# Membrizard/ml_conformer_generator

Hardware: AMD Instinct MI355X
Metric: valid molecules/sec @100 diffusion steps (`value` = RAW molecules/s through the whole public path: the reference's validity gate needs RDKit + trained weights, unavailable offline; see `validity`) (higher is better)
Workload: dtype f32

## Files before the change

### ml_conformer_generator_amd/csrc/mcg_gemm_kernels.h

```cpp
#pragma once
#include "mcg_gemm.h"

#include <type_traits>


__device__ __forceinline__ float* mcg_gemm_c_ptr(const McgGemmArgs& p, int orow, int nt, int g) {
    if (!p.c_blocked) return p.C + (size_t)orow * p.ldc + nt * 16 + 4 * g;
    const int part = nt >= 27 ? 1 : 0, ntp = nt - 27 * part;
    return p.C + ((size_t)((part * 14 + (ntp >> 1)) * 8 + (ntp & 1) * 4 + g) * p.M + orow) * 4;
}

__device__ __forceinline__ void mcg_gemm_side_job(const McgGemmArgs& p, int block) {
    const int idx = block * 256 + (int)threadIdx.x;
    const int v = idx >> 2, comp = idx & 3;
    if (v < p.side_M && comp < 3) {
        const int4 sl = p.side_slots[v];
        p.side_x[(size_t)v * 4 + comp] += (((p.side_u[(size_t)sl.x * 4 + comp] + p.side_u[(size_t)sl.y * 4 + comp]) + p.side_u[(size_t)sl.z * 4 + comp]) +
                                           p.side_u[(size_t)sl.w * 4 + comp]) / 100.0f;
    }
}

template <int RN, int GATHER = 0>
__global__ __launch_bounds__(256) void mcg_gemm_bf16_kernel(McgGemmArgs p) {
    const int lane = threadIdx.x & 63;
// ... 213 lines not shown
            if (k0 + e >= K) v[e] = 0.f;
        typedef __bf16 bf16x4 __attribute__((ext_vector_type(4)));
        const bf16x4 h4 = (bf16x4){(__bf16)v[0], (__bf16)v[1], (__bf16)v[2], (__bf16)v[3]};
        char* dst = reinterpret_cast<char*>(sA) + (((2 * frag_kb + (i >> 1)) * 64 + 16 * (piece >> 1) + 8 * (i & 1) + prow) * 16 + (piece & 1) * 8);
        *reinterpret_cast<bf16x4*>(dst) = h4;
    };
    {
        const __amdgpu_buffer_rsrc_t rs_a1 = __builtin_amdgcn_make_buffer_rsrc(const_cast<float*>(p.A1), 0, 0xffffffff, 0x00020000);
        for (int kb = wid; kb < b1; kb += MCG_LDSG_WAVES) {
            f32x4 v[4];
#pragma unroll
            for (int i = 0; i < 4; ++i) v[i] = __builtin_bit_cast(f32x4, ld(rs_a1, (unsigned)(qrow[i] * p.lda1 + 32 * kb + 4 * piece) * 4u, 0));
#pragma unroll
            for (int i = 0; i < 4; ++i) park_quarter(kb, i, v[i], 32 * kb + 4 * piece, p.K1);
        }
    }
    constexpr int NS = GATHER >= 2 ? GATHER : 1;
    constexpr int S2P = SEG2 ? MCG_LDSG_S2P : 0;
    f32x4 s2[SEG2 ? 2 : 1][4][NS];
    const __amdgpu_buffer_rsrc_t rs_a2 = __builtin_amdgcn_make_buffer_rsrc(const_cast<float*>(p.A2 ? p.A2 : p.A1), 0, 0xffffffff, 0x00020000);
    int srow[4][NS];
#pragma unroll
    for (int i = 0; i < 4; ++i) {
        if constexpr (GATHER >= 2) {
            const int4 sl = (SEG2 && p.a2_rows) ? p.a2_rows[qrow[i]] : (int4){0, 0, 0, 0};
            const int rows[4] = {sl.x, sl.y, sl.z, sl.w};
#pragma unroll
            for (int q = 0; q < NS; ++q) srow[i][q] = rows[q];
        } else {
            srow[i][0] = qrow[i];
        }
    }
    auto seg2_issue = [&](int j) {
        int kb = wid + j * MCG_LDSG_WAVES;
        kb = kb < b2 ? kb : b2 - 1;
#pragma unroll
        for (int i = 0; i < 4; ++i)
#pragma unroll
            for (int q = 0; q < NS; ++q)
                s2[j][i][q] = __builtin_bit_cast(f32x4, ld(rs_a2, (unsigned)(srow[i][q] * p.lda2 + 32 * kb + 4 * piece) * 4u, 0));
    };
    auto seg2_park = [&](int j) {
        const int kb = wid + j * MCG_LDSG_WAVES;
        if (kb >= b2) return;
#pragma unroll
        for (int i = 0; i < 4; ++i) {
            f32x4 v = s2[j][i][0];
            if constexpr (GATHER >= 2) {
#pragma unroll
                for (int q = 1; q < NS; ++q) v += s2[j][i][q];
#pragma unroll
                for (int e = 0; e < 4; ++e) v[e] = mcg_div100(v[e]);
            }
            park_quarter(b1 + kb, i, v, 32 * kb + 4 * piece, p.K2);
        }
    };
    f32x4 eres[RESID ? 2 : 1][RN];
    if constexpr (RESID) {
#pragma unroll
        for (int n = 0; n < RN; ++n) {
            const int col = ncl[n] * 16 + 4 * g;
#pragma unroll
            for (int m = 0; m < 2; ++m) {
                const int orow = row0 + 16 * m + c;
                eres[m][n] = (orow < p.M && col + 3 < p.n_store) ? *reinterpret_cast<const f32x4*>(p.resid + (size_t)orow * p.ldr + col)
                                                                  : (f32x4){0.f, 0.f, 0.f, 0.f};
            }
        }
    }
    constexpr bool OVERLAP2 = SEG2 && GATHER <= 2;
    if (SEG2 && b2 > 0) {
        if constexpr (OVERLAP2) {
#pragma unroll
            for (int j = 0; j < S2P; ++j) seg2_issue(j);
        } else {
#pragma unroll
            for (int j = 0; j < S2P; ++j) { seg2_issue(j); seg2_park(j); }
        }
    }
    asm volatile("s_waitcnt lgkmcnt(0)\n\ts_barrier" ::: "memory");

    f32x4 acc[2][RN];
#pragma unroll
    for (int m = 0; m < 2; ++m)
#pragma unroll
        for (int n = 0; n < RN; ++n) acc[m][n] = (f32x4){0.f, 0.f, 0.f, 0.f};
    auto compute = [&](int slot, int kb) {
        const bf16x8 A0 = sA[(2 * kb) * 64 + lane];
        const bf16x8 A1 = sA[(2 * kb + 1) * 64 + lane];
#pragma unroll
        for (int n = 0; n < RN; ++n) {
            acc[0][n] = mcg_mfma_bf16(Br[slot][n], A0, acc[0][n]);
            acc[1][n] = mcg_mfma_bf16(Br[slot][n], A1, acc[1][n]);
        }
    };
    auto k_loop = [&](int k0, int k1) {
        int kb = k0;
#pragma unroll 1
        for (; kb + RING <= k1; kb += RING) {
#pragma unroll
            for (int r = 0; r < RING; ++r) {
                compute(r, kb + r); __builtin_amdgcn_sched_barrier(0); load_w(r, kb + r + RING); __builtin_amdgcn_sched_barrier(0);
            }
        }
#pragma unroll
        for (int r = 0; r < RING - 1; ++r)
            if (kb + r < k1) compute(r, kb + r);
    };
    if (SEG2 && b2 > 0 && OVERLAP2) {
        k_loop(0, b1);
#pragma unroll
        for (int r = 0; r < RING; ++r) load_w(r, b1 + r);
#pragma unroll
        for (int j = 0; j < S2P; ++j) seg2_park(j);
        asm volatile("s_waitcnt lgkmcnt(0)\n\ts_barrier" ::: "memory");
        k_loop(b1, blocks);
    } else {
        k_loop(0, blocks);
    }

#pragma unroll
    for (int n = 0; n < RN; ++n) {
        if (!nvalid[n]) continue;
        const int col = (nt0 + n) * 16 + 4 * g;
        if (col >= p.n_store) continue;
        const f32x4 ebias = p.bias ? *reinterpret_cast<const f32x4*>(p.bias + col) : (f32x4){0.f, 0.f, 0.f, 0.f};
#pragma unroll
        for (int m = 0; m < 2; ++m) {
            const int orow = row0 + 16 * m + c;
            if (orow >= p.M) continue;
            f32x4 v = acc[m][n] + ebias;
            if (p.act == MCG_ACT_SILU) {
#pragma unroll
                for (int r = 0; r < 4; ++r) v[r] = mcg_silu(v[r]);
            } else if (p.act == MCG_ACT_RELU) {
#pragma unroll
                for (int r = 0; r < 4; ++r) v[r] = fmaxf(v[r], 0.f);
            }
            if constexpr (RESID) v += eres[m][n];
            float* dst = mcg_gemm_c_ptr(p, orow, nt0 + n, g);
            if (col + 3 < p.n_store) {
                *reinterpret_cast<f32x4*>(dst) = v;
            } else {
#pragma unroll
                for (int r = 0; r < 4; ++r)
                    if (col + r < p.n_store) dst[r] = v[r];
            }
        }
    }
}

typedef __bf16 bf16x4 __attribute__((ext_vector_type(4)));

template <int RN>
__global__ __launch_bounds__(256) void mcg_gemm_x6_kernel(McgGemmArgs p) {
    __shared__ __attribute__((aligned(16))) uint16_t a_lds[2 * 2 * 3 * 64 * 8];
    const int lane = threadIdx.x & 63;
    const int wid = __builtin_amdgcn_readfirstlane(threadIdx.x >> 6);
    const int g = lane >> 4, c = lane & 15;
    const int wave_cols = (p.n_tiles + RN - 1) / RN;
    const int col_groups = (wave_cols + 3) / 4;
    const int blk = mcg_xcd_remap(blockIdx.x, gridDim.x);
    const int row0 = (blk / col_groups) * 32;
    const int wcol = (blk % col_groups) * 4 + wid;
    const bool wave_live = wcol < wave_cols;
    const int nt0 = (wave_live ? wcol : wave_cols - 1) * RN;
    bool nvalid[RN];
    int ncl[RN];
#pragma unroll
    for (int n = 0; n < RN; ++n) {
        nvalid[n] = wave_live && nt0 + n < p.n_tiles;
        ncl[n] = nt0 + n < p.n_tiles ? n : 0;
    }
    f32x4 acc[2][RN];
#pragma unroll
    for (int m = 0; m < 2; ++m)
#pragma unroll
        for (int n = 0; n < RN; ++n) acc[m][n] = (f32x4){0.f, 0.f, 0.f, 0.f};
    f32x4 ebias[RN];
    f32x4 eres[2][RN];
#pragma unroll
    for (int n = 0; n < RN; ++n) {
        const int col = (nt0 + ncl[n]) * 16 + 4 * g;
        ebias[n] = p.bias ? *reinterpret_cast<const f32x4*>(p.bias + col) : (f32x4){0.f, 0.f, 0.f, 0.f};
#pragma unroll
        for (int m = 0; m < 2; ++m) {
            const int orow = row0 + 16 * m + c;
            eres[m][n] = (p.resid && orow < p.M && col + 3 < p.n_store) ? *reinterpret_cast<const f32x4*>(p.resid + (size_t)orow * p.ldr + col)
                                                                        : (f32x4){0.f, 0.f, 0.f, 0.f};
        }
    }
    const int my_row = 8 * wid + (lane >> 3), my_k = 4 * (lane & 7);
    const int src_row = row0 + my_row < p.M ? row0 + my_row : p.M - 1;
    const int frag_off = (((my_row >> 4) * 3) * 64 + ((my_k >> 3) * 16 + (my_row & 15))) * 8 + (my_k & 7);

    const uint16_t* bseg = reinterpret_cast<const uint16_t*>(p.Bp);
    int stage = 0;
#pragma unroll 1
    for (int seg = 0; seg < 2; ++seg) {
        const float* A = seg == 0 ? p.A1 : p.A2;
        const int K = seg == 0 ? p.K1 : p.K2;
        const int lda = seg == 0 ? p.lda1 : p.lda2;
        if (K == 0) continue;
        const int blocks = mcg_kblocks16(K);
        const __amdgpu_buffer_rsrc_t rs_a = __builtin_amdgcn_make_buffer_rsrc(const_cast<float*>(A), 0, 0xffffffff, 0x00020000);
        const __amdgpu_buffer_rsrc_t rs_b = __builtin_amdgcn_make_buffer_rsrc(const_cast<uint16_t*>(bseg), 0, 0xffffffff, 0x00020000);
        const unsigned oa = (unsigned)(src_row * lda + my_k) * 4u;
        unsigned obn[RN];
#pragma unroll
        for (int n = 0; n < RN; ++n) obn[n] = (unsigned)((nt0 + ncl[n]) * 64 + lane) * 16u;
        const int part_bytes = p.n_tiles * 64 * 16;
        auto ld = [](const __amdgpu_buffer_rsrc_t& r, unsigned v, int so) { return __builtin_amdgcn_raw_buffer_load_b128(r, (int)v, so, 0); };
        auto load_a = [&](int kb) { return __builtin_bit_cast(f32x4, ld(rs_a, oa, 128 * (kb < blocks ? kb : blocks - 1))); };
        bf16x8 Br[2][3][RN];
        auto load_b = [&](int slot, int kb) {
            kb = kb < blocks ? kb : blocks - 1;
#pragma unroll
            for (int q = 0; q < 3; ++q)
#pragma unroll
                for (int n = 0; n < RN; ++n) Br[slot][q][n] = __builtin_bit_cast(bf16x8, ld(rs_b, obn[n], (kb * 3 + q) * part_bytes));
        };
        auto split_store = [&](f32x4 v, int half) {
            uint16_t* dst = a_lds + half * (2 * 3 * 64 * 8) + frag_off;
#pragma unroll
            for (int q = 0; q < 3; ++q) {
                bf16x4 part;
#pragma unroll
                for (int j = 0; j < 4; ++j) part[j] = (__bf16)v[j];
                *reinterpret_cast<bf16x4*>(dst + q * 64 * 8) = part;
                if (q < 2) {
#pragma unroll
                    for (int j = 0; j < 4; ++j) v[j] -= (float)part[j];
                }
            }
        };
        __syncthreads();
        split_store(load_a(0), stage & 1);
        f32x4 a_pref = load_a(1);
        load_b(0, 0);
        load_b(1, 1);
        auto block = [&](int slot, int kb) {
            const int half = (stage + kb) & 1;
            asm volatile("s_waitcnt lgkmcnt(0)" ::: "memory");
            asm volatile("s_barrier" ::: "memory");
            const f32x4 an = a_pref;
            a_pref = load_a(kb + 2);
            __builtin_amdgcn_sched_barrier(0);
            const bf16x8* la = reinterpret_cast<const bf16x8*>(a_lds) + half * (2 * 3 * 64) + lane;
#pragma unroll
            for (int m = 0; m < 2; ++m) {
                bf16x8 af[3];
#pragma unroll
                for (int q = 0; q < 3; ++q) af[q] = la[(m * 3 + q) * 64];
#pragma unroll
                for (int q = 0; q < 3; ++q)
#pragma unroll
                    for (int r = 0; r < 3 - q; ++r)
#pragma unroll
                        for (int n = 0; n < RN; ++n) acc[m][n] = mcg_mfma_bf16(Br[slot][q][n], af[r], acc[m][n]);
            }
            __builtin_amdgcn_sched_barrier(0);
            load_b(slot, kb + 2);
            __builtin_amdgcn_sched_barrier(0);
            split_store(an, half ^ 1);
            __builtin_amdgcn_sched_barrier(0);
        };
        int kb = 0;
#pragma unroll 1
        for (; kb + 2 <= blocks; kb += 2) { block(0, kb); block(1, kb + 1); }
        if (kb < blocks) block(0, kb);
        stage += blocks;
        bseg += mcg_pack16x3_elems(K, p.n_tiles);
    }
#pragma unroll
    for (int n = 0; n < RN; ++n) {
        if (!nvalid[n]) continue;
        const int col = (nt0 + n) * 16 + 4 * g;
        if (col >= p.n_store) continue;
#pragma unroll
        for (int m = 0; m < 2; ++m) {
            const int orow = row0 + 16 * m + c;
            if (orow >= p.M) continue;
            f32x4 v = acc[m][n] + ebias[n];
            if (p.act == MCG_ACT_SILU) {
#pragma unroll
                for (int r = 0; r < 4; ++r) v[r] = mcg_silu(v[r]);
            } else if (p.act == MCG_ACT_RELU) {
#pragma unroll
                for (int r = 0; r < 4; ++r) v[r] = fmaxf(v[r], 0.f);
            }
            v += eres[m][n];
            float* dst = p.C + (size_t)orow * p.ldc + col;
            if (col + 3 < p.n_store) {
                *reinterpret_cast<f32x4*>(dst) = v;
            } else {
#pragma unroll
                for (int r = 0; r < 4; ++r)
                    if (col + r < p.n_store) dst[r] = v[r];
            }
        }
    }
}

template <int RN, int RING = 3>
__global__ __launch_bounds__(256) void mcg_gemm_kernel(McgGemmArgs p) {
    const int lane = threadIdx.x & 63;
    const int wid = threadIdx.x >> 6;
    const int g = lane >> 4, c = lane & 15;
    const int wave_cols = (p.n_tiles + RN - 1) / RN;
    const int nblk = p.gemm_blocks > 0 ? p.gemm_blocks : (int)gridDim.x;
    if ((int)blockIdx.x >= nblk) { mcg_gemm_side_job(p, (int)blockIdx.x - nblk); return; }
    const int wlin = mcg_xcd_remap(blockIdx.x, nblk) * 4 + wid;
    if (wlin >= ((p.M + 31) / 32) * wave_cols) return;
    const int row0 = (wlin / wave_cols) * 32;
    const int nt0 = (wlin % wave_cols) * RN;
    int rA[2];
#pragma unroll
    for (int m = 0; m < 2; ++m) {
        const int r = row0 + 16 * m + c;
        rA[m] = r < p.M ? r : p.M - 1;
    }
    bool nvalid[RN];
    int ncl[RN];
#pragma unroll
    for (int n = 0; n < RN; ++n) {
        nvalid[n] = nt0 + n < p.n_tiles;
        ncl[n] = nvalid[n] ? n : 0;
    }

    f32x4 acc[2][RN];
#pragma unroll
    for (int m = 0; m < 2; ++m)
#pragma unroll
        for (int n = 0; n < RN; ++n) acc[m][n] = (f32x4){0.f, 0.f, 0.f, 0.f};

    f32x4 ebias[RN];
    f32x4 eres[2][RN];
#pragma unroll
    for (int n = 0; n < RN; ++n) {
        const int col = (nt0 + ncl[n]) * 16 + 4 * g;
        ebias[n] = p.bias ? *reinterpret_cast<const f32x4*>(p.bias + col) : (f32x4){0.f, 0.f, 0.f, 0.f};
#pragma unroll
        for (int m = 0; m < 2; ++m) {
            const int orow = row0 + 16 * m + c;
            eres[m][n] = (p.resid && orow < p.M && col + 3 < p.n_store) ? *reinterpret_cast<const f32x4*>(p.resid + (size_t)orow * p.ldr + col)
                                                                        : (f32x4){0.f, 0.f, 0.f, 0.f};
        }
    }

    const float* bseg = p.Bp;
#pragma unroll 1
    for (int seg = 0; seg < 2; ++seg) {
        const float* A = seg == 0 ? p.A1 : p.A2;
        const int K = seg == 0 ? p.K1 : p.K2;
        const int lda = seg == 0 ? p.lda1 : p.lda2;
        if (K == 0) continue;
        const float* a0 = A + (size_t)rA[0] * lda + 4 * g;
        const float* a1 = A + (size_t)rA[1] * lda + 4 * g;
        const int groups = K / 16;
        const size_t gstride = (size_t)p.n_tiles * 256;
        const float* bq = bseg + (size_t)nt0 * 256 + lane * 4;
        if (groups == 0) goto tail_steps;
        {

        f32x4 Ar[RING][2], Br[RING][RN];
        const __amdgpu_buffer_rsrc_t rs_a = __builtin_amdgcn_make_buffer_rsrc(const_cast<float*>(A), 0, 0xffffffff, 0x00020000);
        const __amdgpu_buffer_rsrc_t rs_b = __builtin_amdgcn_make_buffer_rsrc(const_cast<float*>(bseg), 0, 0xffffffff, 0x00020000);
        const unsigned oa0 = (unsigned)(rA[0] * lda + 4 * g) * 4u, oa1 = (unsigned)(rA[1] * lda + 4 * g) * 4u;
        unsigned obn[RN];
#pragma unroll
        for (int n = 0; n < RN; ++n) obn[n] = (unsigned)((nt0 + ncl[n]) * 256 + lane * 4) * 4u;
        const int gbytes = p.n_tiles * 256 * 4;
        auto load_group = [&](int slot, int q) {
            q = q < groups ? q : groups - 1;
            Ar[slot][0] = __builtin_bit_cast(f32x4, __builtin_amdgcn_raw_buffer_load_b128(rs_a, (int)oa0, 64 * q, 0));
            Ar[slot][1] = __builtin_bit_cast(f32x4, __builtin_amdgcn_raw_buffer_load_b128(rs_a, (int)oa1, 64 * q, 0));
#pragma unroll
            for (int n = 0; n < RN; ++n)
                Br[slot][n] = __builtin_bit_cast(f32x4, __builtin_amdgcn_raw_buffer_load_b128(rs_b, (int)obn[n], q * gbytes, 0));
        };
        auto compute = [&](int slot) {
#pragma unroll
            for (int s = 0; s < 4; ++s)
#pragma unroll
                for (int m = 0; m < 2; ++m)
#pragma unroll
                    for (int n = 0; n < RN; ++n) acc[m][n] = mcg_mfma(Br[slot][n][s], Ar[slot][m][s], acc[m][n]);
        };
#pragma unroll
        for (int i = 0; i < RING; ++i) load_group(i, i);
        int q = 0;
#pragma unroll 1
        for (; q + RING <= groups; q += RING) {
#pragma unroll
            for (int i = 0; i < RING; ++i) {
                compute(i); __builtin_amdgcn_sched_barrier(0); load_group(i, q + RING + i); __builtin_amdgcn_sched_barrier(0);
            }
        }
#pragma unroll
        for (int i = 0; i < RING - 1; ++i)
            if (q + i < groups) compute(i);
        }
    tail_steps:
        const int tail = (K - groups * 16) / 4;
        const float* bt = bseg + (size_t)groups * gstride + (size_t)nt0 * 64 + lane;
        for (int st = 0; st < tail; ++st) {
            const float av0 = a0[groups * 16 + 4 * st - 4 * g + g];
            const float av1 = a1[groups * 16 + 4 * st - 4 * g + g];
#pragma unroll
            for (int n = 0; n < RN; ++n) {
                const float b = bt[(size_t)st * p.n_tiles * 64 + ncl[n] * 64];
                acc[0][n] = mcg_mfma(b, av0, acc[0][n]);
                acc[1][n] = mcg_mfma(b, av1, acc[1][n]);
            }
        }
        bseg += mcg_pack4_floats(K, p.n_tiles);
    }

#pragma unroll
    for (int n = 0; n < RN; ++n) {
        if (!nvalid[n]) continue;
        const int col = (nt0 + n) * 16 + 4 * g;
        if (col >= p.n_store) continue;
#pragma unroll
        for (int m = 0; m < 2; ++m) {
            const int orow = row0 + 16 * m + c;
            if (orow >= p.M) continue;
            f32x4 v = acc[m][n] + ebias[n];
            if (p.act == MCG_ACT_SILU) {
#pragma unroll
                for (int r = 0; r < 4; ++r) v[r] = mcg_silu(v[r]);
            } else if (p.act == MCG_ACT_RELU) {
#pragma unroll
                for (int r = 0; r < 4; ++r) v[r] = fmaxf(v[r], 0.f);
            }
            v += eres[m][n];
            float* dst = mcg_gemm_c_ptr(p, orow, nt0 + n, g);
            if (col + 3 < p.n_store) {
                *reinterpret_cast<f32x4*>(dst) = v;
            } else {
#pragma unroll
                for (int r = 0; r < 4; ++r)
                    if (col + r < p.n_store) dst[r] = v[r];
            }
        }
    }
}


template <int RN, int GATHER, int MR = 1, int RING = 3>
__global__ __launch_bounds__(256) void mcg_gemm16_kernel(McgGemmArgs p) {
    if ((int)blockIdx.x >= p.gemm_blocks) { mcg_gemm_side_job(p, (int)blockIdx.x - p.gemm_blocks); return; }
    const int lane = threadIdx.x & 63;
    const int wid = threadIdx.x >> 6;
    const int g = lane >> 4, c = lane & 15;
    const int wave_cols = (p.n_tiles + RN - 1) / RN;
    const int wlin = mcg_xcd_remap(blockIdx.x, p.gemm_blocks) * 4 + wid;
    if (wlin >= ((p.M + 16 * MR - 1) / (16 * MR)) * wave_cols) return;
    const int row0 = (wlin / wave_cols) * 16 * MR;
    const int nt0 = (wlin % wave_cols) * RN;
    int orow[MR], rA[MR];
#pragma unroll
    for (int m = 0; m < MR; ++m) {
        orow[m] = row0 + 16 * m + c;
        rA[m] = orow[m] < p.M ? orow[m] : p.M - 1;
    }
    bool nvalid[RN];
    int ncl[RN];
#pragma unroll
    for (int n = 0; n < RN; ++n) {
        nvalid[n] = nt0 + n < p.n_tiles;
        ncl[n] = nvalid[n] ? n : 0;
    }
    f32x4 acc[MR][RN];
#pragma unroll
    for (int m = 0; m < MR; ++m)
#pragma unroll
        for (int n = 0; n < RN; ++n) acc[m][n] = (f32x4){0.f, 0.f, 0.f, 0.f};
    f32x4 ebias[RN], eres[MR][RN];
#pragma unroll
    for (int n = 0; n < RN; ++n) {
        const int col = (nt0 + ncl[n]) * 16 + 4 * g;
        ebias[n] = p.bias ? *reinterpret_cast<const f32x4*>(p.bias + col) : (f32x4){0.f, 0.f, 0.f, 0.f};
#pragma unroll
        for (int m = 0; m < MR; ++m)
            eres[m][n] = (p.resid && orow[m] < p.M && col + 3 < p.n_store) ? *reinterpret_cast<const f32x4*>(p.resid + (size_t)orow[m] * p.ldr + col)
                                                                            : (f32x4){0.f, 0.f, 0.f, 0.f};
    }
    const float* bseg = p.Bp;
    auto segment = [&](auto nsum_tag, const float* A, int K, int lda, const int (&ra)[MR], const int (&rb)[MR], const int (&rc)[MR],
                       const int (&rd)[MR]) {
        constexpr int NSUM = decltype(nsum_tag)::value;
        constexpr bool TWO = NSUM >= 2, THREE = NSUM >= 3, FOUR = NSUM >= 4;
        const int groups = K / 16;
        const size_t gstride = (size_t)p.n_tiles * 256;
        if (groups > 0) {
            f32x4 Ar[RING][MR], Ar2[RING][MR], Ar3[RING][MR], Ar4[RING][MR], Br[RING][RN];
            const __amdgpu_buffer_rsrc_t rs_a = __builtin_amdgcn_make_buffer_rsrc(const_cast<float*>(A), 0, 0xffffffff, 0x00020000);
            const __amdgpu_buffer_rsrc_t rs_b = __builtin_amdgcn_make_buffer_rsrc(const_cast<float*>(bseg), 0, 0xffffffff, 0x00020000);
            unsigned oa[MR], oa2[MR], oa3[MR], oa4[MR];
#pragma unroll
            for (int m = 0; m < MR; ++m) {
                oa[m] = (unsigned)(ra[m] * lda + 4 * g) * 4u; oa2[m] = (unsigned)(rb[m] * lda + 4 * g) * 4u; oa3[m] = (unsigned)(rc[m] * lda + 4 * g) * 4u;
                oa4[m] = (unsigned)(rd[m] * lda + 4 * g) * 4u;
            }
            unsigned obn[RN];
#pragma unroll
            for (int n = 0; n < RN; ++n) obn[n] = (unsigned)((nt0 + ncl[n]) * 256 + lane * 4) * 4u;
            const int gbytes = p.n_tiles * 256 * 4;
            auto load_group = [&](int slot, int q) {
                q = q < groups ? q : groups - 1;
#pragma unroll
                for (int m = 0; m < MR; ++m) {
                    Ar[slot][m] = __builtin_bit_cast(f32x4, __builtin_amdgcn_raw_buffer_load_b128(rs_a, (int)oa[m], 64 * q, 0));
                    if (TWO) Ar2[slot][m] = __builtin_bit_cast(f32x4, __builtin_amdgcn_raw_buffer_load_b128(rs_a, (int)oa2[m], 64 * q, 0));
                    if (THREE) Ar3[slot][m] = __builtin_bit_cast(f32x4, __builtin_amdgcn_raw_buffer_load_b128(rs_a, (int)oa3[m], 64 * q, 0));
                    if (FOUR) Ar4[slot][m] = __builtin_bit_cast(f32x4, __builtin_amdgcn_raw_buffer_load_b128(rs_a, (int)oa4[m], 64 * q, 0));
                }
#pragma unroll
                for (int n = 0; n < RN; ++n)
                    Br[slot][n] = __builtin_bit_cast(f32x4, __builtin_amdgcn_raw_buffer_load_b128(rs_b, (int)obn[n], q * gbytes, 0));
            };
            auto compute = [&](int slot) {
                f32x4 a[MR];
#pragma unroll
                for (int m = 0; m < MR; ++m)
                    a[m] = FOUR ? ((Ar[slot][m] + Ar2[slot][m]) + Ar3[slot][m]) + Ar4[slot][m]
                         : THREE ? (Ar[slot][m] + Ar2[slot][m]) + Ar3[slot][m] : TWO ? Ar[slot][m] + Ar2[slot][m] : Ar[slot][m];
#pragma unroll
                for (int s = 0; s < 4; ++s)
#pragma unroll
                    for (int m = 0; m < MR; ++m)
#pragma unroll
                        for (int n = 0; n < RN; ++n) acc[m][n] = mcg_mfma(Br[slot][n][s], a[m][s], acc[m][n]);
            };
#pragma unroll
            for (int i = 0; i < RING; ++i) load_group(i, i);
            int q = 0;
#pragma unroll 1
            for (; q + RING <= groups; q += RING) {
#pragma unroll
                for (int i = 0; i < RING; ++i) {
                    compute(i); __builtin_amdgcn_sched_barrier(0); load_group(i, q + RING + i); __builtin_amdgcn_sched_barrier(0);
                }
            }
#pragma unroll
            for (int i = 0; i < RING - 1; ++i)
                if (q + i < groups) compute(i);
        }
        const int tail = (K - groups * 16) / 4;
        const float* bt = bseg + (size_t)groups * gstride + (size_t)nt0 * 64 + lane;
        for (int st = 0; st < tail; ++st) {
            const int k = groups * 16 + 4 * st + g;
            float av[MR];
#pragma unroll
            for (int m = 0; m < MR; ++m) {
                av[m] = A[(size_t)ra[m] * lda + k];
                if (TWO) av[m] += A[(size_t)rb[m] * lda + k];
                if (THREE) av[m] += A[(size_t)rc[m] * lda + k];
                if (FOUR) av[m] += A[(size_t)rd[m] * lda + k];
            }
#pragma unroll
            for (int n = 0; n < RN; ++n) {
                const float b = bt[(size_t)st * p.n_tiles * 64 + ncl[n] * 64];
#pragma unroll
                for (int m = 0; m < MR; ++m) acc[m][n] = mcg_mfma(b, av[m], acc[m][n]);
            }
        }
        bseg += mcg_pack4_floats(K, p.n_tiles);
    };
    if (p.K1 > 0) segment(std::integral_constant<int, 1>{}, p.A1, p.K1, p.lda1, rA, rA, rA, rA);
    if (p.K2 > 0) {
        if (GATHER) {
            int sa[MR], sb[MR], sc[MR], sd[MR];
#pragma unroll
            for (int m = 0; m < MR; ++m) { const int4 sl = p.a2_rows[rA[m]]; sa[m] = sl.x; sb[m] = sl.y; sc[m] = sl.z; sd[m] = sl.w; }
            segment(std::integral_constant<int, (GATHER >= 2 ? GATHER : 1)>{}, p.A2, p.K2, p.lda2, sa, sb, sc, sd);
        } else {
            segment(std::integral_constant<int, 1>{}, p.A2, p.K2, p.lda2, rA, rA, rA, rA);
        }
    }
#pragma unroll
    for (int n = 0; n < RN; ++n) {
        if (!nvalid[n]) continue;
        const int col = (nt0 + n) * 16 + 4 * g;
        if (col >= p.n_store) continue;
#pragma unroll
        for (int m = 0; m < MR; ++m) {
            if (orow[m] >= p.M) continue;
            f32x4 v = acc[m][n] + ebias[n];
            if (p.act == MCG_ACT_SILU) {
#pragma unroll
                for (int r = 0; r < 4; ++r) v[r] = mcg_silu(v[r]);
            } else if (p.act == MCG_ACT_RELU) {
#pragma unroll
                for (int r = 0; r < 4; ++r) v[r] = fmaxf(v[r], 0.f);
            }
            v += eres[m][n];
            float* dst = p.C + (size_t)orow[m] * p.ldc + col;
            if (col + 3 < p.n_store) {
                *reinterpret_cast<f32x4*>(dst) = v;
            } else {
#pragma unroll
                for (int r = 0; r < 4; ++r)
                    if (col + r < p.n_store) dst[r] = v[r];
            }
        }
    }
}
```

Baseline: 139.6.

## Unify f32 GEMM kernels into one tile routine with cross-segment prefetch pipeline

Merges the two f32 MFMA GEMM kernels into a shared tile function. The K1 and K2 segments now run as one continuous ring-buffered pipeline, so K2 loads are issued while K1 is still computing. Tail loads and the bias/residual epilogue loads are issued early to hide their latency. Buffer descriptors with a zero num_records (through an s_ashr trick) let out-of-range prefetches return zero instead of being clamped. This adds complexity and register pressure, and relies on buffer out-of-bounds semantics for correctness.

Result: faster. 141.5 (median of 6 runs) (+1.3%).

```diff
diff --git a/ml_conformer_generator_amd/csrc/mcg_gemm_kernels.h b/ml_conformer_generator_amd/csrc/mcg_gemm_kernels.h
--- a/ml_conformer_generator_amd/csrc/mcg_gemm_kernels.h
+++ b/ml_conformer_generator_amd/csrc/mcg_gemm_kernels.h
@@ -539,309 +539,265 @@
     }
 }
 
+template <int RN, int GATHER, int MR, int RING, bool C_PTR>
+__device__ __forceinline__ void mcg_gemm_f32_tile(const McgGemmArgs& p, int row0, int nt0) {
+    constexpr int NS = GATHER >= 2 ? GATHER : 1;
+    const int lane = threadIdx.x & 63;
+    const int g = lane >> 4, c = lane & 15;
+    int orow[MR], rA[MR];
+#pragma unroll
+    for (int m = 0; m < MR; ++m) {
+        orow[m] = row0 + 16 * m + c;
+        rA[m] = orow[m] < p.M ? orow[m] : p.M - 1;
+    }
+    int4 sl[MR];
+    if constexpr (GATHER >= 2) {
+#pragma unroll
+        for (int m = 0; m < MR; ++m) sl[m] = p.a2_rows[rA[m]];
+    }
+    bool nvalid[RN];
+    int ncl[RN];
+#pragma unroll
+    for (int n = 0; n < RN; ++n) {
+        nvalid[n] = nt0 + n < p.n_tiles;
+        ncl[n] = nvalid[n] ? n : 0;
+    }
+    f32x4 acc[MR][RN];
+#pragma unroll
+    for (int m = 0; m < MR; ++m)
+#pragma unroll
+        for (int n = 0; n < RN; ++n) acc[m][n] = (f32x4){0.f, 0.f, 0.f, 0.f};
+
+    const int G1 = p.K1 / 16, T1 = (p.K1 - 16 * G1) / 4;
+    const int G2 = p.K2 / 16, T2 = (p.K2 - 16 * G2) / 4;
+    const int gbytes = p.n_tiles * 1024;
+    const int b2off = (p.K1 / 4) * p.n_tiles * 256;
+    const __amdgpu_buffer_rsrc_t rs_a1 = __builtin_amdgcn_make_buffer_rsrc(const_cast<float*>(p.A1), 0, 0xffffffff, 0x00020000);
+    const __amdgpu_buffer_rsrc_t rs_a2 = __builtin_amdgcn_make_buffer_rsrc(const_cast<float*>(p.A2), 0, 0xffffffff, 0x00020000);
+    const __amdgpu_buffer_rsrc_t rs_b = __builtin_amdgcn_make_buffer_rsrc(const_cast<float*>(p.Bp), 0, 0xffffffff, 0x00020000);
+    int n1, n2;
+    asm("s_ashr_i32 %0, %1, 31" : "=s"(n1) : "s"(-G1) : "scc");
+    asm("s_ashr_i32 %0, %1, 31" : "=s"(n2) : "s"(-G2) : "scc");
+    const __amdgpu_buffer_rsrc_t rg_a1 = __builtin_amdgcn_make_buffer_rsrc(const_cast<float*>(p.A1), 0, n1, 0x00020000);
+    const __amdgpu_buffer_rsrc_t rg_b1 = __builtin_amdgcn_make_buffer_rsrc(const_cast<float*>(p.Bp), 0, n1, 0x00020000);
+    const __amdgpu_buffer_rsrc_t rg_a2 = __builtin_amdgcn_make_buffer_rsrc(const_cast<float*>(p.A2), 0, n2, 0x00020000);
+    const __amdgpu_buffer_rsrc_t rg_b2 = __builtin_amdgcn_make_buffer_rsrc(const_cast<float*>(p.Bp), 0, n2, 0x00020000);
+    auto ld4 = [](const __amdgpu_buffer_rsrc_t& r, unsigned v, int so) { return __builtin_bit_cast(f32x4, __builtin_amdgcn_raw_buffer_load_b128(r, (int)v, so, 0)); };
+    auto ld1 = [](const __amdgpu_buffer_rsrc_t& r, unsigned v, int so) { return __builtin_bit_cast(float, __builtin_amdgcn_raw_buffer_load_b32(r, (int)v, so, 0)); };
+    unsigned oa1[MR], ob[RN];
+#pragma unroll
+    for (int m = 0; m < MR; ++m) oa1[m] = (unsigned)(rA[m] * p.lda1 + 4 * g) * 4u;
+#pragma unroll
+    for (int n = 0; n < RN; ++n) ob[n] = (unsigned)((nt0 + ncl[n]) * 256 + lane * 4) * 4u;
+
+    float ta1[3][MR], tb1[3][RN], ta2[3][MR][NS], tb2[3][RN];
+#pragma unroll
+    for (int st = 0; st < 3; ++st) {
+#pragma unroll
+        for (int n = 0; n < RN; ++n) tb1[st][n] = tb2[st][n] = 0.f;
+#pragma unroll
+        for (int m = 0; m < MR; ++m) {
+            ta1[st][m] = 0.f;
+#pragma unroll
+            for (int q = 0; q < NS; ++q) ta2[st][m][q] = 0.f;
+        }
+    }
+#pragma unroll
+    for (int st = 0; st < 3; ++st)
+        if (st < T1) {
+#pragma unroll
+            for (int m = 0; m < MR; ++m) ta1[st][m] = ld1(rs_a1, oa1[m] - 12u * g, (16 * G1 + 4 * st) * 4);
+#pragma unroll
+            for (int n = 0; n < RN; ++n) tb1[st][n] = ld1(rs_b, ob[n] >> 2, G1 * gbytes + st * (gbytes >> 2));
+        }
+
+    f32x4 Ar[RING][MR][NS], Br[RING][RN];
+    unsigned oa2[MR][NS];
+    auto load1 = [&](int slot, int q) {
+#pragma unroll
+        for (int m = 0; m < MR; ++m) Ar[slot][m][0] = ld4(rg_a1, oa1[m], 64 * q);
+#pragma unroll
+        for (int n = 0; n < RN; ++n) Br[slot][n] = ld4(rg_b1, ob[n], q * gbytes);
+    };
+    auto load2 = [&](int slot, int q) {
+        q = q < G2 ? q : G2 - 1;
+#pragma unroll
+        for (int m = 0; m < MR; ++m)
+#pragma unroll
+            for (int s = 0; s < NS; ++s) Ar[slot][m][s] = ld4(rg_a2, oa2[m][s], 64 * q);
+#pragma unroll
+        for (int n = 0; n < RN; ++n) Br[slot][n] = ld4(rg_b2, ob[n], b2off + q * gbytes);
+    };
+    auto mfmas = [&](int slot, const f32x4 (&a)[MR]) {
+#pragma unroll
+        for (int s = 0; s < 4; ++s)
+#pragma unroll
+            for (int m = 0; m < MR; ++m)
+#pragma unroll
+                for (int n = 0; n < RN; ++n) acc[m][n] = mcg_mfma(Br[slot][n][s], a[m][s], acc[m][n]);
+    };
+    auto compute1 = [&](int slot) {
+        f32x4 a[MR];
+#pragma unroll
+        for (int m = 0; m < MR; ++m) a[m] = Ar[slot][m][0];
+        mfmas(slot, a);
+    };
+    auto compute2 = [&](int slot) {
+        f32x4 a[MR];
+#pragma unroll
+        for (int m = 0; m < MR; ++m) {
+            a[m] = Ar[slot][m][0];
+#pragma unroll
+            for (int s = 1; s < NS; ++s) a[m] = a[m] + Ar[slot][m][s];
+        }
+        mfmas(slot, a);
+    };
+    const int s0 = G1 > 0 ? (RING - G1 % RING) % RING : RING;
+#pragma unroll
+    for (int i = 0; i < RING; ++i) { load1(i, __builtin_amdgcn_readfirstlane(i > s0 ? i - s0 : 0)); __builtin_amdgcn_sched_barrier(0); }
+    __builtin_amdgcn_sched_barrier(0);
+
+    f32x4 ebias[RN], eres[MR][RN];
+#pragma unroll
+    for (int n = 0; n < RN; ++n) {
+        const int col = (nt0 + ncl[n]) * 16 + 4 * g;
+        ebias[n] = p.bias ? *reinterpret_cast<const f32x4*>(p.bias + col) : (f32x4){0.f, 0.f, 0.f, 0.f};
+#pragma unroll
+        for (int m = 0; m < MR; ++m)
+            eres[m][n] = (p.resid && orow[m] < p.M && col + 3 < p.n_store) ? *reinterpret_cast<const f32x4*>(p.resid + (size_t)orow[m] * p.ldr + col)
+                                                                            : (f32x4){0.f, 0.f, 0.f, 0.f};
+    }
+    __builtin_amdgcn_sched_barrier(0);
+
+#pragma unroll
+    for (int m = 0; m < MR; ++m) {
+        if constexpr (GATHER >= 2) {
+            const int rows[4] = {sl[m].x, sl[m].y, sl[m].z, sl[m].w};
+#pragma unroll
+            for (int s = 0; s < NS; ++s) oa2[m][s] = (unsigned)(rows[s] * p.lda2 + 4 * g) * 4u;
+        } else {
+            oa2[m][0] = (unsigned)(rA[m] * p.lda2 + 4 * g) * 4u;
+        }
+    }
+#pragma unroll
+    for (int st = 0; st < 3; ++st)
+        if (st < T2) {
+#pragma unroll
+            for (int m = 0; m < MR; ++m)
+#pragma unroll
+                for (int s = 0; s < NS; ++s) ta2[st][m][s] = ld1(rs_a2, oa2[m][s] - 12u * g, (16 * G2 + 4 * st) * 4);
+#pragma unroll
+            for (int n = 0; n < RN; ++n) tb2[st][n] = ld1(rs_b, ob[n] >> 2, b2off + G2 * gbytes + st * (gbytes >> 2));
+        }
+    __builtin_amdgcn_sched_barrier(0);
+
+    {
+        int b = -s0;
+        if (G1 > RING) {
+#pragma unroll
+            for (int i = 0; i < RING; ++i) {
+                if (b + i >= 0) compute1(i);
+                __builtin_amdgcn_sched_barrier(0); load1(i, b + RING + i); __builtin_amdgcn_sched_barrier(0);
+            }
+            b += RING;
+#pragma unroll 1
+            for (; b + RING < G1; b += RING) {
+#pragma unroll
+                for (int i = 0; i < RING; ++i) {
+                    compute1(i); __builtin_amdgcn_sched_barrier(0); load1(i, b + RING + i); __builtin_amdgcn_sched_barrier(0);
+                }
+            }
+        }
+#pragma unroll
+        for (int i = 0; i < RING; ++i) {
+            if (b + i >= 0) compute1(i);
+            __builtin_amdgcn_sched_barrier(0); load2(i, i); __builtin_amdgcn_sched_barrier(0);
+        }
+    }
+#pragma unroll
+    for (int st = 0; st < 3; ++st)
+        if (st < T1) {
+#pragma unroll
+            for (int n = 0; n < RN; ++n)
+#pragma unroll
+                for (int m = 0; m < MR; ++m) acc[m][n] = mcg_mfma(tb1[st][n], ta1[st][m], acc[m][n]);
+        }
+
+    if (G2 > 0) {
+        int q = 0;
+#pragma unroll 1
+        for (; q + RING <= G2; q += RING) {
+#pragma unroll
+            for (int i = 0; i < RING; ++i) {
+                compute2(i); __builtin_amdgcn_sched_barrier(0); load2(i, q + RING + i); __builtin_amdgcn_sched_barrier(0);
+            }
+        }
+#pragma unroll
+        for (int i = 0; i < RING - 1; ++i)
+            if (q + i < G2) compute2(i);
+    }
+#pragma unroll
+    for (int st = 0; st < 3; ++st)
+        if (st < T2) {
+            float av[MR];
+#pragma unroll
+            for (int m = 0; m < MR; ++m) {
+                av[m] = ta2[st][m][0];
+#pragma unroll
+                for (int s = 1; s < NS; ++s) av[m] += ta2[st][m][s];
+            }
+#pragma unroll
+            for (int n = 0; n < RN; ++n)
+#pragma unroll
+                for (int m = 0; m < MR; ++m) acc[m][n] = mcg_mfma(tb2[st][n], av[m], acc[m][n]);
+        }
+
+#pragma unroll
+    for (int n = 0; n < RN; ++n) {
+        if (!nvalid[n]) continue;
+        const int col = (nt0 + n) * 16 + 4 * g;
+        if (col >= p.n_store) continue;
+#pragma unroll
+        for (int m = 0; m < MR; ++m) {
+            if (orow[m] >= p.M) continue;
+            f32x4 v = acc[m][n] + ebias[n];
+            if (p.act == MCG_ACT_SILU) {
+#pragma unroll
+                for (int r = 0; r < 4; ++r) v[r] = mcg_silu(v[r]);
+            } else if (p.act == MCG_ACT_RELU) {
+#pragma unroll
+                for (int r = 0; r < 4; ++r) v[r] = fmaxf(v[r], 0.f);
+            }
+            v += eres[m][n];
+            float* dst = C_PTR ? mcg_gemm_c_ptr(p, orow[m], nt0 + n, g) : p.C + (size_t)orow[m] * p.ldc + col;
+            if (col + 3 < p.n_store) {
+                *reinterpret_cast<f32x4*>(dst) = v;
+            } else {
+#pragma unroll
+                for (int r = 0; r < 4; ++r)
+                    if (col + r < p.n_store) dst[r] = v[r];
+            }
+        }
+    }
+}
+
 template <int RN, int RING = 3>
 __global__ __launch_bounds__(256) void mcg_gemm_kernel(McgGemmArgs p) {
-    const int lane = threadIdx.x & 63;
     const int wid = threadIdx.x >> 6;
-    const int g = lane >> 4, c = lane & 15;
     const int wave_cols = (p.n_tiles + RN - 1) / RN;
     const int nblk = p.gemm_blocks > 0 ? p.gemm_blocks : (int)gridDim.x;
     if ((int)blockIdx.x >= nblk) { mcg_gemm_side_job(p, (int)blockIdx.x - nblk); return; }
     const int wlin = mcg_xcd_remap(blockIdx.x, nblk) * 4 + wid;
     if (wlin >= ((p.M + 31) / 32) * wave_cols) return;
-    const int row0 = (wlin / wave_cols) * 32;
-    const int nt0 = (wlin % wave_cols) * RN;
-    int rA[2];
-#pragma unroll
-    for (int m = 0; m < 2; ++m) {
-        const int r = row0 + 16 * m + c;
-        rA[m] = r < p.M ? r : p.M - 1;
-    }
-    bool nvalid[RN];
-    int ncl[RN];
-#pragma unroll
-    for (int n = 0; n < RN; ++n) {
-        nvalid[n] = nt0 + n < p.n_tiles;
-        ncl[n] = nvalid[n] ? n : 0;
-    }
-
-    f32x4 acc[2][RN];
-#pragma unroll
-    for (int m = 0; m < 2; ++m)
-#pragma unroll
-        for (int n = 0; n < RN; ++n) acc[m][n] = (f32x4){0.f, 0.f, 0.f, 0.f};
-
-    f32x4 ebias[RN];
-    f32x4 eres[2][RN];
-#pragma unroll
-    for (int n = 0; n < RN; ++n) {
-        const int col = (nt0 + ncl[n]) * 16 + 4 * g;
-        ebias[n] = p.bias ? *reinterpret_cast<const f32x4*>(p.bias + col) : (f32x4){0.f, 0.f, 0.f, 0.f};
-#pragma unroll
-        for (int m = 0; m < 2; ++m) {
-            const int orow = row0 + 16 * m + c;
-            eres[m][n] = (p.resid && orow < p.M && col + 3 < p.n_store) ? *reinterpret_cast<const f32x4*>(p.resid + (size_t)orow * p.ldr + col)
-                                                                        : (f32x4){0.f, 0.f, 0.f, 0.f};
-        }
-    }
-
-    const float* bseg = p.Bp;
-#pragma unroll 1
-    for (int seg = 0; seg < 2; ++seg) {
-        const float* A = seg == 0 ? p.A1 : p.A2;
-        const int K = seg == 0 ? p.K1 : p.K2;
-        const int lda = seg == 0 ? p.lda1 : p.lda2;
-        if (K == 0) continue;
-        const float* a0 = A + (size_t)rA[0] * lda + 4 * g;
-        const float* a1 = A + (size_t)rA[1] * lda + 4 * g;
-        const int groups = K / 16;
-        const size_t gstride = (size_t)p.n_tiles * 256;
-        const float* bq = bseg + (size_t)nt0 * 256 + lane * 4;
-        if (groups == 0) goto tail_steps;
-        {
-
-        f32x4 Ar[RING][2], Br[RING][RN];
-        const __amdgpu_buffer_rsrc_t rs_a = __builtin_amdgcn_make_buffer_rsrc(const_cast<float*>(A), 0, 0xffffffff, 0x00020000);
-        const __amdgpu_buffer_rsrc_t rs_b = __builtin_amdgcn_make_buffer_rsrc(const_cast<float*>(bseg), 0, 0xffffffff, 0x00020000);
-        const unsigned oa0 = (unsigned)(rA[0] * lda + 4 * g) * 4u, oa1 = (unsigned)(rA[1] * lda + 4 * g) * 4u;
-        unsigned obn[RN];
-#pragma unroll
-        for (int n = 0; n < RN; ++n) obn[n] = (unsigned)((nt0 + ncl[n]) * 256 + lane * 4) * 4u;
-        const int gbytes = p.n_tiles * 256 * 4;
-        auto load_group = [&](int slot, int q) {
-            q = q < groups ? q : groups - 1;
-            Ar[slot][0] = __builtin_bit_cast(f32x4, __builtin_amdgcn_raw_buffer_load_b128(rs_a, (int)oa0, 64 * q, 0));
-            Ar[slot][1] = __builtin_bit_cast(f32x4, __builtin_amdgcn_raw_buffer_load_b128(rs_a, (int)oa1, 64 * q, 0));
-#pragma unroll
-            for (int n = 0; n < RN; ++n)
-                Br[slot][n] = __builtin_bit_cast(f32x4, __builtin_amdgcn_raw_buffer_load_b128(rs_b, (int)obn[n], q * gbytes, 0));
-        };
-        auto compute = [&](int slot) {
-#pragma unroll
-            for (int s = 0; s < 4; ++s)
-#pragma unroll
-                for (int m = 0; m < 2; ++m)
-#pragma unroll
-                    for (int n = 0; n < RN; ++n) acc[m][n] = mcg_mfma(Br[slot][n][s], Ar[slot][m][s], acc[m][n]);
-        };
-#pragma unroll
-        for (int i = 0; i < RING; ++i) load_group(i, i);
-        int q = 0;
-#pragma unroll 1
-        for (; q + RING <= groups; q += RING) {
-#pragma unroll
-            for (int i = 0; i < RING; ++i) {
-                compute(i); __builtin_amdgcn_sched_barrier(0); load_group(i, q + RING + i); __builtin_amdgcn_sched_barrier(0);
-            }
-        }
-#pragma unroll
-        for (int i = 0; i < RING - 1; ++i)
-            if (q + i < groups) compute(i);
-        }
-    tail_steps:
-        const int tail = (K - groups * 16) / 4;
-        const float* bt = bseg + (size_t)groups * gstride + (size_t)nt0 * 64 + lane;
-        for (int st = 0; st < tail; ++st) {
-            const float av0 = a0[groups * 16 + 4 * st - 4 * g + g];
-            const float av1 = a1[groups * 16 + 4 * st - 4 * g + g];
-#pragma unroll
-            for (int n = 0; n < RN; ++n) {
-                const float b = bt[(size_t)st * p.n_tiles * 64 + ncl[n] * 64];
-                acc[0][n] = mcg_mfma(b, av0, acc[0][n]);
-                acc[1][n] = mcg_mfma(b, av1, acc[1][n]);
-            }
-        }
-        bseg += mcg_pack4_floats(K, p.n_tiles);
-    }
-
-#pragma unroll
-    for (int n = 0; n < RN; ++n) {
-        if (!nvalid[n]) continue;
-        const int col = (nt0 + n) * 16 + 4 * g;
-        if (col >= p.n_store) continue;
-#pragma unroll
-        for (int m = 0; m < 2; ++m) {
-            const int orow = row0 + 16 * m + c;
-            if (orow >= p.M) continue;
-            f32x4 v = acc[m][n] + ebias[n];
-            if (p.act == MCG_ACT_SILU) {
-#pragma unroll
-                for (int r = 0; r < 4; ++r) v[r] = mcg_silu(v[r]);
-            } else if (p.act == MCG_ACT_RELU) {
-#pragma unroll
-                for (int r = 0; r < 4; ++r) v[r] = fmaxf(v[r], 0.f);
-            }
-            v += eres[m][n];
-            float* dst = mcg_gemm_c_ptr(p, orow, nt0 + n, g);
-            if (col + 3 < p.n_store) {
-                *reinterpret_cast<f32x4*>(dst) = v;
-            } else {
-#pragma unroll
-                for (int r = 0; r < 4; ++r)
-                    if (col + r < p.n_store) dst[r] = v[r];
-            }
-        }
-    }
+    mcg_gemm_f32_tile<RN, 0, 2, RING, true>(p, (wlin / wave_cols) * 32, (wlin % wave_cols) * RN);
 }
-
 
 template <int RN, int GATHER, int MR = 1, int RING = 3>
 __global__ __launch_bounds__(256) void mcg_gemm16_kernel(McgGemmArgs p) {
     if ((int)blockIdx.x >= p.gemm_blocks) { mcg_gemm_side_job(p, (int)blockIdx.x - p.gemm_blocks); return; }
-    const int lane = threadIdx.x & 63;
     const int wid = threadIdx.x >> 6;
-    const int g = lane >> 4, c = lane & 15;
     const int wave_cols = (p.n_tiles + RN - 1) / RN;
     const int wlin = mcg_xcd_remap(blockIdx.x, p.gemm_blocks) * 4 + wid;
     if (wlin >= ((p.M + 16 * MR - 1) / (16 * MR)) * wave_cols) return;
-    const int row0 = (wlin / wave_cols) * 16 * MR;
-    const int nt0 = (wlin % wave_cols) * RN;
-    int orow[MR], rA[MR];
-#pragma unroll
-    for (int m = 0; m < MR; ++m) {
-        orow[m] = row0 + 16 * m + c;
-        rA[m] = orow[m] < p.M ? orow[m] : p.M - 1;
-    }
-    bool nvalid[RN];
-    int ncl[RN];
-#pragma unroll
-    for (int n = 0; n < RN; ++n) {
-        nvalid[n] = nt0 + n < p.n_tiles;
-        ncl[n] = nvalid[n] ? n : 0;
-    }
-    f32x4 acc[MR][RN];
-#pragma unroll
-    for (int m = 0; m < MR; ++m)
-#pragma unroll
-        for (int n = 0; n < RN; ++n) acc[m][n] = (f32x4){0.f, 0.f, 0.f, 0.f};
-    f32x4 ebias[RN], eres[MR][RN];
-#pragma unroll
-    for (int n = 0; n < RN; ++n) {
-        const int col = (nt0 + ncl[n]) * 16 + 4 * g;
-        ebias[n] = p.bias ? *reinterpret_cast<const f32x4*>(p.bias + col) : (f32x4){0.f, 0.f, 0.f, 0.f};
-#pragma unroll
-        for (int m = 0; m < MR; ++m)
-            eres[m][n] = (p.resid && orow[m] < p.M && col + 3 < p.n_store) ? *reinterpret_cast<const f32x4*>(p.resid + (size_t)orow[m] * p.ldr + col)
-                                                                            : (f32x4){0.f, 0.f, 0.f, 0.f};
-    }
-    const float* bseg = p.Bp;
-    auto segment = [&](auto nsum_tag, const float* A, int K, int lda, const int (&ra)[MR], const int (&rb)[MR], const int (&rc)[MR],
-                       const int (&rd)[MR]) {
-        constexpr int NSUM = decltype(nsum_tag)::value;
-        constexpr bool TWO = NSUM >= 2, THREE = NSUM >= 3, FOUR = NSUM >= 4;
-        const int groups = K / 16;
-        const size_t gstride = (size_t)p.n_tiles * 256;
-        if (groups > 0) {
-            f32x4 Ar[RING][MR], Ar2[RING][MR], Ar3[RING][MR], Ar4[RING][MR], Br[RING][RN];
-            const __amdgpu_buffer_rsrc_t rs_a = __builtin_amdgcn_make_buffer_rsrc(const_cast<float*>(A), 0, 0xffffffff, 0x00020000);
-            const __amdgpu_buffer_rsrc_t rs_b = __builtin_amdgcn_make_buffer_rsrc(const_cast<float*>(bseg), 0, 0xffffffff, 0x00020000);
-            unsigned oa[MR], oa2[MR], oa3[MR], oa4[MR];
-#pragma unroll
-            for (int m = 0; m < MR; ++m) {
-                oa[m] = (unsigned)(ra[m] * lda + 4 * g) * 4u; oa2[m] = (unsigned)(rb[m] * lda + 4 * g) * 4u; oa3[m] = (unsigned)(rc[m] * lda + 4 * g) * 4u;
-                oa4[m] = (unsigned)(rd[m] * lda + 4 * g) * 4u;
-            }
-            unsigned obn[RN];
-#pragma unroll
-            for (int n = 0; n < RN; ++n) obn[n] = (unsigned)((nt0 + ncl[n]) * 256 + lane * 4) * 4u;
-            const int gbytes = p.n_tiles * 256 * 4;
-            auto load_group = [&](int slot, int q) {
-                q = q < groups ? q : groups - 1;
-#pragma unroll
-                for (int m = 0; m < MR; ++m) {
-                    Ar[slot][m] = __builtin_bit_cast(f32x4, __builtin_amdgcn_raw_buffer_load_b128(rs_a, (int)oa[m], 64 * q, 0));
-                    if (TWO) Ar2[slot][m] = __builtin_bit_cast(f32x4, __builtin_amdgcn_raw_buffer_load_b128(rs_a, (int)oa2[m], 64 * q, 0));
-                    if (THREE) Ar3[slot][m] = __builtin_bit_cast(f32x4, __builtin_amdgcn_raw_buffer_load_b128(rs_a, (int)oa3[m], 64 * q, 0));
-                    if (FOUR) Ar4[slot][m] = __builtin_bit_cast(f32x4, __builtin_amdgcn_raw_buffer_load_b128(rs_a, (int)oa4[m], 64 * q, 0));
-                }
-#pragma unroll
-                for (int n = 0; n < RN; ++n)
-                    Br[slot][n] = __builtin_bit_cast(f32x4, __builtin_amdgcn_raw_buffer_load_b128(rs_b, (int)obn[n], q * gbytes, 0));
-            };
-            auto compute = [&](int slot) {
-                f32x4 a[MR];
-#pragma unroll
-                for (int m = 0; m < MR; ++m)
-                    a[m] = FOUR ? ((Ar[slot][m] + Ar2[slot][m]) + Ar3[slot][m]) + Ar4[slot][m]
-                         : THREE ? (Ar[slot][m] + Ar2[slot][m]) + Ar3[slot][m] : TWO ? Ar[slot][m] + Ar2[slot][m] : Ar[slot][m];
-#pragma unroll
-                for (int s = 0; s < 4; ++s)
-#pragma unroll
-                    for (int m = 0; m < MR; ++m)
-#pragma unroll
-                        for (int n = 0; n < RN; ++n) acc[m][n] = mcg_mfma(Br[slot][n][s], a[m][s], acc[m][n]);
-            };
-#pragma unroll
-            for (int i = 0; i < RING; ++i) load_group(i, i);
-            int q = 0;
-#pragma unroll 1
-            for (; q + RING <= groups; q += RING) {
-#pragma unroll
-                for (int i = 0; i < RING; ++i) {
-                    compute(i); __builtin_amdgcn_sched_barrier(0); load_group(i, q + RING + i); __builtin_amdgcn_sched_barrier(0);
-                }
-            }
-#pragma unroll
-            for (int i = 0; i < RING - 1; ++i)
-                if (q + i < groups) compute(i);
-        }
-        const int tail = (K - groups * 16) / 4;
-        const float* bt = bseg + (size_t)groups * gstride + (size_t)nt0 * 64 + lane;
-        for (int st = 0; st < tail; ++st) {
-            const int k = groups * 16 + 4 * st + g;
-            float av[MR];
-#pragma unroll
-            for (int m = 0; m < MR; ++m) {
-                av[m] = A[(size_t)ra[m] * lda + k];
-                if (TWO) av[m] += A[(size_t)rb[m] * lda + k];
-                if (THREE) av[m] += A[(size_t)rc[m] * lda + k];
-                if (FOUR) av[m] += A[(size_t)rd[m] * lda + k];
-            }
-#pragma unroll
-            for (int n = 0; n < RN; ++n) {
-                const float b = bt[(size_t)st * p.n_tiles * 64 + ncl[n] * 64];
-#pragma unroll
-                for (int m = 0; m < MR; ++m) acc[m][n] = mcg_mfma(b, av[m], acc[m][n]);
-            }
-        }
-        bseg += mcg_pack4_floats(K, p.n_tiles);
-    };
-    if (p.K1 > 0) segment(std::integral_constant<int, 1>{}, p.A1, p.K1, p.lda1, rA, rA, rA, rA);
-    if (p.K2 > 0) {
-        if (GATHER) {
-            int sa[MR], sb[MR], sc[MR], sd[MR];
-#pragma unroll
-            for (int m = 0; m < MR; ++m) { const int4 sl = p.a2_rows[rA[m]]; sa[m] = sl.x; sb[m] = sl.y; sc[m] = sl.z; sd[m] = sl.w; }
-            segment(std::integral_constant<int, (GATHER >= 2 ? GATHER : 1)>{}, p.A2, p.K2, p.lda2, sa, sb, sc, sd);
-        } else {
-            segment(std::integral_constant<int, 1>{}, p.A2, p.K2, p.lda2, rA, rA, rA, rA);
-        }
-    }
-#pragma unroll
-    for (int n = 0; n < RN; ++n) {
-        if (!nvalid[n]) continue;
-        const int col = (nt0 + n) * 16 + 4 * g;
-        if (col >= p.n_store) continue;
-#pragma unroll
-        for (int m = 0; m < MR; ++m) {
-            if (orow[m] >= p.M) continue;
-            f32x4 v = acc[m][n] + ebias[n];
-            if (p.act == MCG_ACT_SILU) {
-#pragma unroll
-                for (int r = 0; r < 4; ++r) v[r] = mcg_silu(v[r]);
-            } else if (p.act == MCG_ACT_RELU) {
-#pragma unroll
-                for (int r = 0; r < 4; ++r) v[r] = fmaxf(v[r], 0.f);
-            }
-            v += eres[m][n];
-            float* dst = p.C + (size_t)orow[m] * p.ldc + col;
-            if (col + 3 < p.n_store) {
-                *reinterpret_cast<f32x4*>(dst) = v;
-            } else {
-#pragma unroll
-                for (int r = 0; r < 4; ++r)
-                    if (col + r < p.n_store) dst[r] = v[r];
-            }
-        }
-    }
+    mcg_gemm_f32_tile<RN, GATHER, MR, RING, false>(p, (wlin / wave_cols) * 16 * MR, (wlin % wave_cols) * RN);
 }
```
